# josebeo2016/SCL-Deepfake-audio-detection

Hardware: AMD Instinct MI355X
Metric: train-step utterances/sec (64000-sample clips) (higher is better)
Workload: dtype bf16

## Files before the change

scl-deepfake-audio-detection_amd/csrc/conv0.hip:

```cpp
#include "common.h"

namespace {

constexpr int MAXK = 16;
constexpr int MAXCH0 = 2;

struct Conv0Smem {
    float* wT;
    float* xs;
    float* red;
};

__device__ __forceinline__ void conv0_stage(float* wT, float* xs, const float* __restrict__ w, const float* __restrict__ x,
                                            int C, int k, int L, int x0, int nx) {
    for (int i = threadIdx.x; i < C * k; i += blockDim.x) {
        const int c = i / k, j = i % k;
        wT[j * C + c] = w[i];
    }
    for (int i = threadIdx.x; i < nx; i += blockDim.x) xs[i] = (x0 + i) < L ? x[x0 + i] : 0.f;
}

template <bool ZF32, int KC>
__global__ __launch_bounds__(256) void conv0_fwd_kernel(const float* __restrict__ x, const float* __restrict__ w,
                                                        const float* __restrict__ bias, const float* __restrict__ gamma,
                                                        const float* __restrict__ beta, void* __restrict__ zv, float* __restrict__ stats,
                                                        int L, int T0, int C, int k, int stride, int rows_per_block, float eps) {
    extern __shared__ __attribute__((aligned(16))) float sm0[];
    float* wT = sm0;
    float* xs = sm0 + k * C;
    const int b = blockIdx.y;
    const int t0 = blockIdx.x * rows_per_block;
    const int nrows = min(rows_per_block, T0 - t0);
    const int nx = nrows * stride + k;
    conv0_stage(wT, xs, w, x + (int64_t)b * L, C, k, L, t0 * stride, nx);
    __syncthreads();
    const int lane = threadIdx.x & 63, wv = threadIdx.x >> 6;
    float bia[MAXCH0][8], gam[MAXCH0][8], bet[MAXCH0][8];
#pragma unroll
    for (int ch = 0; ch < MAXCH0; ++ch) {
        const int c = ch * 512 + lane * 8;
#pragma unroll
        for (int i = 0; i < 8; ++i) {
            bia[ch][i] = c < C ? bias[c + i] : 0.f; gam[ch][i] = c < C ? gamma[c + i] : 0.f; bet[ch][i] = c < C ? beta[c + i] : 0.f;
        }
    }
    for (int r = wv; r < nrows; r += 4) {
        float y[MAXCH0][8];
        float s = 0.f;
#pragma unroll
        for (int ch = 0; ch < MAXCH0; ++ch) {
            const int c = ch * 512 + lane * 8;
            if (c < C) {
#pragma unroll
                for (int i = 0; i < 8; ++i) y[ch][i] = bia[ch][i];
#pragma unroll
                for (int j = 0; j < (KC ? KC : k); ++j) {
                    const float xv = xs[r * stride + j];
                    const float4 w0 = *reinterpret_cast<const float4*>(wT + j * C + c);
                    const float4 w1 = *reinterpret_cast<const float4*>(wT + j * C + c + 4);
                    y[ch][0] += w0.x * xv; y[ch][1] += w0.y * xv; y[ch][2] += w0.z * xv; y[ch][3] += w0.w * xv;
                    y[ch][4] += w1.x * xv; y[ch][5] += w1.y * xv; y[ch][6] += w1.z * xv; y[ch][7] += w1.w * xv;
                }
#pragma unroll
                for (int i = 0; i < 8; ++i) s += y[ch][i];
            }
        }
        const float mean = wave_sum(s) / (float)C;
        float q = 0.f;
#pragma unroll
        for (int ch = 0; ch < MAXCH0; ++ch) {
            const int c = ch * 512 + lane * 8;
            if (c < C) {
#pragma unroll
                for (int i = 0; i < 8; ++i) { const float d = y[ch][i] - mean; q += d * d; }
            }
        }
        const float rstd = rsqrtf(wave_sum(q) / (float)C + eps);
        if (stats && lane == 0) {
            stats[2 * ((int64_t)b * T0 + t0 + r)] = mean;
            stats[2 * ((int64_t)b * T0 + t0 + r) + 1] = rstd;
        }
#pragma unroll
        for (int ch = 0; ch < MAXCH0; ++ch) {
            const int c = ch * 512 + lane * 8;
            if (c < C) {
                float o[8];
#pragma unroll
                for (int i = 0; i < 8; ++i) o[i] = (y[ch][i] - mean) * rstd * gam[ch][i] + bet[ch][i];
#pragma unroll
                for (int i = 0; i < 8; i += 2) gelu2(o[i], o[i + 1]);
                const int64_t off = ((int64_t)b * T0 + t0 + r) * C + c;
                if (ZF32) {
                    float* z = reinterpret_cast<float*>(zv);
                    *reinterpret_cast<float4*>(z + off) = make_float4(o[0], o[1], o[2], o[3]);
                    *reinterpret_cast<float4*>(z + off + 4) = make_float4(o[4], o[5], o[6], o[7]);
                } else {
                    uint4 u;
                    u.x = pack_bf2(o[0], o[1]); u.y = pack_bf2(o[2], o[3]); u.z = pack_bf2(o[4], o[5]); u.w = pack_bf2(o[6], o[7]);
                    *reinterpret_cast<uint4*>(reinterpret_cast<bf16_t*>(zv) + off) = u;
                }
            }
        }
    }
}

template <bool STATS, int KT, bool FULLK>
__global__ __launch_bounds__(256, 2) void conv0_bwd_kernel(const float* __restrict__ x, const float* __restrict__ w,
                                                           const float* __restrict__ bias, const float* __restrict__ gamma,
                                                           const float* __restrict__ beta, const bf16_t* __restrict__ dz,
                                                           const float* __restrict__ stats, float* __restrict__ part, int L, int T0, int C,
                                                           int k, int stride, int rows_per_block, float eps) {
    extern __shared__ __attribute__((aligned(16))) float sm0[];
    float* wT = sm0;
    float* xs = sm0 + k * C;
    float* red = sm0;
    const int b = blockIdx.y;
    const int t0 = blockIdx.x * rows_per_block;
    const int nrows = min(rows_per_block, T0 - t0);
    const int nx = nrows * stride + k;
    conv0_stage(wT, xs, w, x + (int64_t)b * L, C, k, L, t0 * stride, nx);
    __syncthreads();
    const int lane = threadIdx.x & 63, wv = threadIdx.x >> 6;
    float aw[8][KT + 3];
#pragma unroll
    for (int i = 0; i < 8; ++i)
#pragma unroll
        for (int q = 0; q < KT + 3; ++q) aw[i][q] = 0.f;
    const int c = lane * 8;
    const bool act = c < C;
    float gam[8], bet[8], bia[8];
#pragma unroll
    for (int i = 0; i < 8; ++i) { gam[i] = act ? gamma[c + i] : 0.f; bet[i] = act ? beta[c + i] : 0.f; bia[i] = act ? bias[c + i] : 0.f; }
    uint4 u_next = make_uint4(0, 0, 0, 0);
    float mean_next = 0.f, rstd_next = 0.f;
    if (wv < nrows) {
        const int64_t row0 = (int64_t)b * T0 + t0 + wv;
        if (act) u_next = *reinterpret_cast<const uint4*>(dz + row0 * C + c);
        if (STATS) { mean_next = stats[2 * row0]; rstd_next = stats[2 * row0 + 1]; }
    }
    for (int r = wv; r < nrows; r += 4) {
        float y[8], g8[8], dzv[8], xr[KT];
        const int64_t row = (int64_t)b * T0 + t0 + r;
        const uint4 u = u_next;
        const float mean_cur = mean_next, rstd_cur = rstd_next;
        if (r + 4 < nrows) {
            if (act) u_next = *reinterpret_cast<const uint4*>(dz + (row + 4) * C + c);
            if (STATS) { mean_next = stats[2 * (row + 4)]; rstd_next = stats[2 * (row + 4) + 1]; }
        }
#pragma unroll
        for (int j = 0; j < KT; ++j) xr[j] = (FULLK || j < k) ? xs[r * stride + j] : 0.f;
        if (act) {
#pragma unroll
            for (int i = 0; i < 8; ++i) y[i] = bia[i];
#pragma unroll
            for (int j = 0; j < KT; ++j) {
                if (j < k) {
                    const float4 w0 = *reinterpret_cast<const float4*>(wT + j * C + c);
                    const float4 w1 = *reinterpret_cast<const float4*>(wT + j * C + c + 4);
                    y[0] += w0.x * xr[j]; y[1] += w0.y * xr[j]; y[2] += w0.z * xr[j]; y[3] += w0.w * xr[j];
                    y[4] += w1.x * xr[j]; y[5] += w1.y * xr[j]; y[6] += w1.z * xr[j]; y[7] += w1.w * xr[j];
                }

            }
            const uint32_t uw[4] = {u.x, u.y, u.z, u.w};
#pragma unroll
            for (int i = 0; i < 4; ++i) { dzv[2 * i] = __uint_as_float(uw[i] << 16); dzv[2 * i + 1] = __uint_as_float(uw[i] & 0xFFFF0000u); }
        } else {
#pragma unroll
            for (int i = 0; i < 8; ++i) { y[i] = 0.f; dzv[i] = 0.f; }
        }
        float mean, rstd;
        if (STATS) {
            mean = mean_cur; rstd = rstd_cur;
        } else {
            float s = 0.f;
#pragma unroll
            for (int i = 0; i < 8; ++i) s += y[i];
            mean = wave_sum(s) / (float)C;
            float q = 0.f;
            if (act) {
#pragma unroll
                for (int i = 0; i < 8; ++i) { const float dd = y[i] - mean; q += dd * dd; }
            }
            rstd = rsqrtf(wave_sum(q) / (float)C + eps);
        }
        float s1 = 0.f, s2 = 0.f;
        if (act) {
            float gg[8];
#pragma unroll
            for (int i = 0; i < 8; ++i) gg[i] = ((y[i] - mean) * rstd) * gam[i] + bet[i];
#pragma unroll
            for (int i = 0; i < 8; i += 2) gelu_grad2(gg[i], gg[i + 1]);
#pragma unroll
            for (int i = 0; i < 8; ++i) {
                const float h = (y[i] - mean) * rstd;
                const float gmi = gam[i];
                const float dyn = dzv[i] * gg[i];
                aw[i][KT + 1] += dyn * h;
                aw[i][KT + 2] += dyn;
                const float dh = dyn * gmi;
                y[i] = h;
                g8[i] = dh;
                s1 += dh; s2 += dh * h;
            }
        }
        s1 = wave_sum(s1) / (float)C;
        s2 = wave_sum(s2) / (float)C;
        if (act) {
#pragma unroll
            for (int i = 0; i < 8; ++i) {
                const float dy = rstd * (g8[i] - s1 - y[i] * s2);
                aw[i][KT] += dy;
#pragma unroll
                for (int j = 0; j < KT; ++j)
                    if (FULLK || j < k) aw[i][j] += dy * xr[j];
            }
        }
    }
    __syncthreads();
    for (int i = threadIdx.x; i < C * (k + 3); i += blockDim.x) red[i] = 0.f;
    __syncthreads();
    for (int ww = 0; ww < 4; ++ww) {
        if (wv == ww && act) {
#pragma unroll
            for (int i = 0; i < 8; ++i) {
#pragma unroll
                for (int j = 0; j < KT; ++j)
                    if (FULLK || j < k) red[(c + i) * (k + 3) + j] += aw[i][j];
                red[(c + i) * (k + 3) + k] += aw[i][KT];
                red[(c + i) * (k + 3) + k + 1] += aw[i][KT + 1];
                red[(c + i) * (k + 3) + k + 2] += aw[i][KT + 2];
            }
        }
        __syncthreads();
    }
    const int64_t blk = (int64_t)blockIdx.y * gridDim.x + blockIdx.x;
    for (int i = threadIdx.x; i < C * (k + 3); i += blockDim.x) part[blk * C * (k + 3) + i] = red[i];
}

__global__ void conv0_reduce_seg_kernel(float* __restrict__ part, int nparts, int n, int S) {
    const int i = blockIdx.x * blockDim.x + threadIdx.x;
    const int g = blockIdx.y;
    if (i >= n || g >= nparts) return;
    float s = 0.f;
    for (int p = g; p < nparts; p += S) s += part[(int64_t)p * n + i];
    part[(int64_t)g * n + i] = s;
}

__global__ void conv0_reduce_kernel(const float* __restrict__ part, int nparts, int C, int k, float* __restrict__ dW,
                                    float* __restrict__ db, float* __restrict__ dgamma, float* __restrict__ dbeta) {
    const int i = blockIdx.x * blockDim.x + threadIdx.x;
    const int n = C * (k + 3);
    if (i >= n) return;
    float s = 0.f;
    for (int p = 0; p < nparts; ++p) s += part[(int64_t)p * n + i];
    const int c = i / (k + 3), q = i % (k + 3);
    if (q < k) dW[c * k + q] = s;
    else if (q == k) db[c] = s;
    else if (q == k + 1) dgamma[c] = s;
    else dbeta[c] = s;
}

}

static int conv0_bwd_rows(int B, int T0) {
    int best_rows = 1024; long long best = -1;
    for (int chunks = (T0 + 1023) / 1024; chunks <= (T0 + 63) / 64; ++chunks) {
        const int rows = (T0 + chunks - 1) / chunks;
        const long long blocks = (long long)B * ((T0 + rows - 1) / rows);
        const long long cost = ((blocks + 511) / 512) * (rows + 48);
        if (best < 0 || cost < best) { best = cost; best_rows = rows; }
        if (blocks > 8192) break;
    }
    return best_rows < 64 ? 64 : best_rows;
}

extern "C" int scl_conv0_fwd(const float* x, const float* w, const float* bias, const float* gamma, const float* beta,
                             void* z, float* stats, int B, int L, int C, int k, int stride, float eps, void* stream) {
    SCL_REQUIRE(x && w && bias && gamma && beta && z, "conv0_fwd: null pointer");
    SCL_REQUIRE(B > 0 && L >= k && C >= 8 && C <= 1024 && (C & 7) == 0 && k >= 1 && k <= MAXK && stride >= 1, "conv0_fwd: bad dims");
    const int T0 = (L - k) / stride + 1;
    const int rows = 128;
    dim3 grid((T0 + rows - 1) / rows, B), block(256);
    const size_t lds = (size_t)(k * C + rows * stride + k) * sizeof(float);
    if (k == 10) hipLaunchKernelGGL((conv0_fwd_kernel<false, 10>), grid, block, lds, (hipStream_t)stream, x, w, bias, gamma, beta, z, stats, L, T0, C, k, stride, rows, eps);
    else hipLaunchKernelGGL((conv0_fwd_kernel<false, 0>), grid, block, lds, (hipStream_t)stream, x, w, bias, gamma, beta, z, stats, L, T0, C, k, stride, rows, eps);
    return scl_check_launch("scl_conv0_fwd");
}

extern "C" int scl_conv0_fwd_f32(const float* x, const float* w, const float* bias, const float* gamma, const float* beta,
                                 float* z, int B, int L, int C, int k, int stride, float eps, void* stream) {
    SCL_REQUIRE(x && w && bias && gamma && beta && z, "conv0_fwd_f32: null pointer");
    SCL_REQUIRE(B > 0 && L >= k && C >= 8 && C <= 1024 && (C & 7) == 0 && k >= 1 && k <= MAXK && stride >= 1, "conv0_fwd_f32: bad dims");
    const int T0 = (L - k) / stride + 1;
    const int rows = 128;
    dim3 grid((T0 + rows - 1) / rows, B), block(256);
    const size_t lds = (size_t)(k * C + rows * stride + k) * sizeof(float);
    if (k == 10) hipLaunchKernelGGL((conv0_fwd_kernel<true, 10>), grid, block, lds, (hipStream_t)stream, x, w, bias, gamma, beta, (void*)z, nullptr, L, T0, C, k, stride, rows, eps);
    else hipLaunchKernelGGL((conv0_fwd_kernel<true, 0>), grid, block, lds, (hipStream_t)stream, x, w, bias, gamma, beta, (void*)z, nullptr, L, T0, C, k, stride, rows, eps);
    return scl_check_launch("scl_conv0_fwd_f32");
}

extern "C" int scl_conv0_bwd_nparts(int B, int L, int k, int stride) {
    const int T0 = (L - k) / stride + 1;
    const int rows = conv0_bwd_rows(B, T0);
    return B * ((T0 + rows - 1) / rows);
}

extern "C" int scl_conv0_bwd(const float* x, const float* w, const float* bias, const float* gamma, const float* beta,
                             const void* dz, const float* stats, float* part_ws, float* dW, float* db, float* dgamma, float* dbeta,
                             int B, int L, int C, int k, int stride, float eps, void* stream) {
    SCL_REQUIRE(x && w && bias && gamma && beta && dz && part_ws && dW && db && dgamma && dbeta, "conv0_bwd: null pointer");
    SCL_REQUIRE(B > 0 && L >= k && C >= 8 && C <= 512 && (C & 7) == 0 && k >= 1 && k <= MAXK && stride >= 1, "conv0_bwd: bad dims (C <= 512)");
    const int T0 = (L - k) / stride + 1;
    const int rows = conv0_bwd_rows(B, T0);
    dim3 grid((T0 + rows - 1) / rows, B), block(256);
    const size_t a = (size_t)(k * C + rows * stride + k), r = (size_t)C * (k + 3);
    const size_t lds = (a > r ? a : r) * sizeof(float);
    hipStream_t s = (hipStream_t)stream;
#define CONV0_BWD(ST, KT, FK) hipLaunchKernelGGL((conv0_bwd_kernel<ST, KT, FK>), grid, block, lds, s, x, w, bias, gamma, beta, (const bf16_t*)dz, stats, \
                                                 part_ws, L, T0, C, k, stride, rows, eps)
    if (k == 10) { if (stats) CONV0_BWD(true, 10, true); else CONV0_BWD(false, 10, true); }
    else if (k < 10) { if (stats) CONV0_BWD(true, 10, false); else CONV0_BWD(false, 10, false); }
    else { if (stats) CONV0_BWD(true, MAXK, false); else CONV0_BWD(false, MAXK, false); }
#undef CONV0_BWD
    int nparts = grid.x * grid.y;
    const int n = C * (k + 3);
    if (nparts > 64) {
        const int S = 32;
        hipLaunchKernelGGL(conv0_reduce_seg_kernel, dim3((n + 255) / 256, S), dim3(256), 0, s, part_ws, nparts, n, S);
        nparts = S;
    }
    hipLaunchKernelGGL(conv0_reduce_kernel, dim3((n + 255) / 256), dim3(256), 0, s, part_ws, nparts, C, k, dW, db, dgamma, dbeta);
    return scl_check_launch("scl_conv0_bwd");
}
```

Measured before the change: 1633.

## Add MFMA-based conv0 forward and backward kernels with fused LayerNorm and GELU

Adds new first-layer conv kernels for forward and backward that compute the k-tap convolution as fp32 MFMA 16x16x4 matrix ops, using a rearranged weight layout in shared memory. LayerNorm, GELU and the parameter gradients stay fused in the same kernel. The backward kernel splits channels across waves and exchanges row sums through LDS, and the forward picks its row tiling from a cost model. This moves conv0 work off scalar FMAs onto the matrix units. The path is on by default and can be turned off with an environment variable. It adds a lot of code and uses an erf approximation for GELU, which carries some numerical risk.

```diff
diff --git a/scl-deepfake-audio-detection_amd/csrc/conv0.hip b/scl-deepfake-audio-detection_amd/csrc/conv0.hip
--- a/scl-deepfake-audio-detection_amd/csrc/conv0.hip
+++ b/scl-deepfake-audio-detection_amd/csrc/conv0.hip
@@ -1,3 +1,4 @@
+#include <stdlib.h>
 #include "common.h"
 
 namespace {
@@ -105,7 +106,7 @@
 }
 
 template <bool STATS, int KT, bool FULLK>
-__global__ __launch_bounds__(256, 2) void conv0_bwd_kernel(const float* __restrict__ x, const float* __restrict__ w,
+__global__ __launch_bounds__(256, KT > 10 ? 1 : 2) void conv0_bwd_kernel(const float* __restrict__ x, const float* __restrict__ w,
                                                            const float* __restrict__ bias, const float* __restrict__ gamma,
                                                            const float* __restrict__ beta, const bf16_t* __restrict__ dz,
                                                            const float* __restrict__ stats, float* __restrict__ part, int L, int T0, int C,
@@ -261,6 +262,361 @@
     else dbeta[c] = s;
 }
 
+constexpr int C0M_PAD = 16;
+
+__device__ __forceinline__ int conv0m_channel(int t, int n) { return 128 * (t >> 3) + 8 * n + (t & 7); }
+__device__ __forceinline__ int conv0m_slab(int rows, int stride) { return ((rows + 15) & ~15) * stride + C0M_PAD; }
+
+__device__ __forceinline__ void conv0m_stage(float* wB, float* xs, const float* __restrict__ w, const float* __restrict__ x,
+                                             int C, int k, int nm, int L, int x0, int nx) {
+    const int nt4 = C >> 6;
+    for (int i = threadIdx.x; i < nm * C * 4; i += blockDim.x) {
+        const int e = i & 3, ln = (i >> 2) & 63, rest = i >> 8;
+        const int t = 4 * (rest % nt4) + e, m = rest / nt4;
+        const int tap = 4 * m + (ln >> 4);
+        wB[i] = tap < k ? w[conv0m_channel(t, ln & 15) * k + tap] : 0.f;
+    }
+    for (int i = threadIdx.x; i < nx; i += blockDim.x) xs[i] = (x0 + i) < L ? x[x0 + i] : 0.f;
+}
+
+template <int NV>
+__device__ __forceinline__ void conv0m_gelu_parts(const float (&x)[NV], float (&cdf)[NV], float (&e)[NV]) {
+#pragma clang fp contract(off)
+    typedef __attribute__((ext_vector_type(NV))) float vec;
+    vec xv, ax, t, ev;
+#pragma unroll
+    for (int i = 0; i < NV; ++i) { xv[i] = x[i]; ax[i] = fabsf(x[i]); }
+    const vec z = ax * 0.70710678118654752f;
+    const vec den = __builtin_elementwise_fma(vec(0.3275911f), z, vec(1.0f));
+#pragma unroll
+    for (int i = 0; i < NV; ++i) t[i] = __builtin_amdgcn_rcpf(den[i]);
+    const vec z2 = z * z;
+#pragma unroll
+    for (int i = 0; i < NV; ++i) ev[i] = __expf(-z2[i]);
+    vec p = __builtin_elementwise_fma(t, vec(1.061405429f), vec(-1.453152027f));
+    p = __builtin_elementwise_fma(t, p, vec(1.421413741f));
+    p = __builtin_elementwise_fma(t, p, vec(-0.284496736f));
+    p = __builtin_elementwise_fma(t, p, vec(0.254829592f));
+    const vec half_tail = (0.5f * (t * p)) * ev;
+#pragma unroll
+    for (int i = 0; i < NV; ++i) { cdf[i] = x[i] >= 0.f ? 1.0f - half_tail[i] : half_tail[i]; e[i] = ev[i]; }
+}
+template <int NV>
+__device__ __forceinline__ void conv0m_gelu(float (&x)[NV]) {
+    float cdf[NV], e[NV];
+    conv0m_gelu_parts<NV>(x, cdf, e);
+#pragma unroll
+    for (int i = 0; i < NV; ++i) x[i] = x[i] * cdf[i];
+}
+template <int NV>
+__device__ __forceinline__ void conv0m_gelu_grad(float (&x)[NV]) {
+#pragma clang fp contract(off)
+    float cdf[NV], e[NV];
+    conv0m_gelu_parts<NV>(x, cdf, e);
+#pragma unroll
+    for (int i = 0; i < NV; ++i) x[i] = __builtin_fmaf(x[i] * 0.39894228040143268f, e[i], cdf[i]);
+}
+
+template <bool ZF32, int NC, int KM>
+__global__ __launch_bounds__(256, 2) void conv0_fwd_mfma_kernel(const float* __restrict__ x, const float* __restrict__ w,
+                                                                const float* __restrict__ bias, const float* __restrict__ gamma,
+                                                                const float* __restrict__ beta, void* __restrict__ zv,
+                                                                float* __restrict__ stats, int L, int T0, int k, int stride,
+                                                                int rows_per_block, float eps) {
+    constexpr int C = 128 * NC, NT = 8 * NC;
+    extern __shared__ __attribute__((aligned(16))) float sm0[];
+    constexpr int nm = KM;
+    float* wB = sm0;
+    float* aff = wB + nm * C * 4;
+    float* xs = aff + 3 * C;
+    const int b = blockIdx.y;
+    const int t0 = blockIdx.x * rows_per_block;
+    const int nrows = min(rows_per_block, T0 - t0);
+    conv0m_stage(wB, xs, w, x + (int64_t)b * L, C, k, nm, L, t0 * stride, conv0m_slab(rows_per_block, stride));
+    for (int i = threadIdx.x; i < C; i += blockDim.x) { aff[i] = bias[i]; aff[C + i] = gamma[i]; aff[2 * C + i] = beta[i]; }
+    __syncthreads();
+    const int lane = threadIdx.x & 63, wv = threadIdx.x >> 6;
+    const int n = lane & 15, g = lane >> 4;
+    const int ngroups = (nrows + 15) >> 4;
+    for (int grp = wv; grp < ngroups; grp += 4) {
+        f32x4 acc[NT];
+#pragma unroll
+        for (int q = 0; q < NC; ++q) {
+            const float4 b0 = *reinterpret_cast<const float4*>(aff + 128 * q + 8 * n);
+            const float4 b1 = *reinterpret_cast<const float4*>(aff + 128 * q + 8 * n + 4);
+            const float bb[8] = {b0.x, b0.y, b0.z, b0.w, b1.x, b1.y, b1.z, b1.w};
+#pragma unroll
+            for (int i = 0; i < 8; ++i) acc[8 * q + i] = f32x4{bb[i], bb[i], bb[i], bb[i]};
+        }
+        const float* xa = xs + stride * (16 * grp + n) + g;
+        const float4* wb = reinterpret_cast<const float4*>(wB) + lane;
+#pragma unroll 1
+        for (int m = 0; m < KM; ++m) {
+            const float a = xa[4 * m];
+#pragma unroll
+            for (int t4 = 0; t4 < NT / 4; ++t4) {
+                const float4 bv = wb[(m * (NT / 4) + t4) * 64];
+                acc[4 * t4 + 0] = __builtin_amdgcn_mfma_f32_16x16x4f32(a, bv.x, acc[4 * t4 + 0], 0, 0, 0);
+                acc[4 * t4 + 1] = __builtin_amdgcn_mfma_f32_16x16x4f32(a, bv.y, acc[4 * t4 + 1], 0, 0, 0);
+                acc[4 * t4 + 2] = __builtin_amdgcn_mfma_f32_16x16x4f32(a, bv.z, acc[4 * t4 + 2], 0, 0, 0);
+                acc[4 * t4 + 3] = __builtin_amdgcn_mfma_f32_16x16x4f32(a, bv.w, acc[4 * t4 + 3], 0, 0, 0);
+            }
+        }
+        float mean[4], rstd[4];
+#pragma unroll
+        for (int r = 0; r < 4; ++r) {
+            float s = 0.f;
+#pragma unroll
+            for (int t = 0; t < NT; ++t) s += acc[t][r];
+            mean[r] = lanes16_sum(s) / (float)C;
+        }
+#pragma unroll
+        for (int r = 0; r < 4; ++r) {
+            float q = 0.f;
+#pragma unroll
+            for (int t = 0; t < NT; ++t) { const float d = acc[t][r] - mean[r]; q += d * d; }
+            rstd[r] = rsqrtf(lanes16_sum(q) / (float)C + eps);
+        }
+        const int fl0 = 16 * grp + 4 * g;
+        const int64_t row0 = (int64_t)b * T0 + t0 + fl0;
+        if (stats && n == 0) {
+#pragma unroll
+            for (int r = 0; r < 4; ++r)
+                if (fl0 + r < nrows) *reinterpret_cast<float2*>(stats + 2 * (row0 + r)) = make_float2(mean[r], rstd[r]);
+        }
+#pragma unroll
+        for (int q = 0; q < NC; ++q) {
+            __builtin_amdgcn_sched_barrier(0);
+            const float4 g0 = *reinterpret_cast<const float4*>(aff + C + 128 * q + 8 * n);
+            const float4 g1 = *reinterpret_cast<const float4*>(aff + C + 128 * q + 8 * n + 4);
+            const float4 e0 = *reinterpret_cast<const float4*>(aff + 2 * C + 128 * q + 8 * n);
+            const float4 e1 = *reinterpret_cast<const float4*>(aff + 2 * C + 128 * q + 8 * n + 4);
+            const float gam[8] = {g0.x, g0.y, g0.z, g0.w, g1.x, g1.y, g1.z, g1.w};
+            const float bet[8] = {e0.x, e0.y, e0.z, e0.w, e1.x, e1.y, e1.z, e1.w};
+#pragma unroll
+            for (int r = 0; r < 4; ++r) {
+                float o[8];
+#pragma unroll
+                for (int i = 0; i < 8; ++i) o[i] = (acc[8 * q + i][r] - mean[r]) * rstd[r] * gam[i] + bet[i];
+                conv0m_gelu<8>(o);
+                if (fl0 + r < nrows) {
+                    const int64_t off = (row0 + r) * C + 128 * q + 8 * n;
+                    if (ZF32) {
+                        float* z = reinterpret_cast<float*>(zv);
+                        *reinterpret_cast<float4*>(z + off) = make_float4(o[0], o[1], o[2], o[3]);
+                        *reinterpret_cast<float4*>(z + off + 4) = make_float4(o[4], o[5], o[6], o[7]);
+                    } else {
+                        uint4 u;
+                        u.x = pack_bf2(o[0], o[1]); u.y = pack_bf2(o[2], o[3]); u.z = pack_bf2(o[4], o[5]); u.w = pack_bf2(o[6], o[7]);
+                        *reinterpret_cast<uint4*>(reinterpret_cast<bf16_t*>(zv) + off) = u;
+                    }
+                }
+            }
+        }
+    }
+}
+
+template <int NC, int KM>
+__global__ __launch_bounds__(64 * NC, 2) void conv0_bwd_mfma_kernel(const float* __restrict__ x, const float* __restrict__ w,
+                                                                    const float* __restrict__ bias, const float* __restrict__ gamma,
+                                                                    const float* __restrict__ beta, const bf16_t* __restrict__ dz,
+                                                                    const float* __restrict__ stats, float* __restrict__ part, int L,
+                                                                    int T0, int k, int stride, int rows_per_block) {
+    constexpr int C = 128 * NC;
+    extern __shared__ __attribute__((aligned(16))) float sm0[];
+    constexpr int nm = KM;
+    float* wB = sm0;
+    float* aff = wB + nm * C * 4;
+    float* ex = aff + 3 * C;
+    float* xs = ex + 2 * NC * 32;
+    const int b = blockIdx.y;
+    const int t0 = blockIdx.x * rows_per_block;
+    const int nrows = min(rows_per_block, T0 - t0);
+    conv0m_stage(wB, xs, w, x + (int64_t)b * L, C, k, nm, L, t0 * stride, conv0m_slab(rows_per_block, stride));
+    for (int i = threadIdx.x; i < C; i += blockDim.x) { aff[i] = bias[i]; aff[C + i] = gamma[i]; aff[2 * C + i] = beta[i]; }
+    __syncthreads();
+    const int lane = threadIdx.x & 63, wv = threadIdx.x >> 6;
+    const int n = lane & 15, g = lane >> 4;
+    const int cb = 128 * wv + 8 * n;
+    f32x4 dwT[8];
+    float adb[8], adg[8], adbe[8];
+#pragma unroll
+    for (int i = 0; i < 8; ++i) { dwT[i] = f32x4{0.f, 0.f, 0.f, 0.f}; adb[i] = 0.f; adg[i] = 0.f; adbe[i] = 0.f; }
+    const int ngroups = (nrows + 15) >> 4;
+    const int64_t rowb = (int64_t)b * T0 + t0;
+    uint4 u[4];
+    float2 st[4];
+#pragma unroll
+    for (int r = 0; r < 4; ++r) {
+        const int fl = 4 * g + r;
+        u[r] = make_uint4(0, 0, 0, 0); st[r] = make_float2(0.f, 0.f);
+        if (fl < nrows) {
+            u[r] = *reinterpret_cast<const uint4*>(dz + (rowb + fl) * C + cb);
+            st[r] = *reinterpret_cast<const float2*>(stats + 2 * (rowb + fl));
+        }
+    }
+    const float4* wb = reinterpret_cast<const float4*>(wB) + lane;
+    for (int grp = 0; grp < ngroups; ++grp) {
+        f32x4 y[8], d[8];
+        {
+            const float4 b0 = *reinterpret_cast<const float4*>(aff + cb), b1 = *reinterpret_cast<const float4*>(aff + cb + 4);
+            const float bia[8] = {b0.x, b0.y, b0.z, b0.w, b1.x, b1.y, b1.z, b1.w};
+#pragma unroll
+            for (int i = 0; i < 8; ++i) y[i] = f32x4{bia[i], bia[i], bia[i], bia[i]};
+        }
+        const float* xa = xs + stride * (16 * grp + n) + g;
+#pragma unroll 1
+        for (int m = 0; m < KM; ++m) {
+            const float a = xa[4 * m];
+            const float4 b0 = wb[(m * 2 * NC + 2 * wv) * 64], b1 = wb[(m * 2 * NC + 2 * wv + 1) * 64];
+            y[0] = __builtin_amdgcn_mfma_f32_16x16x4f32(a, b0.x, y[0], 0, 0, 0);
+            y[1] = __builtin_amdgcn_mfma_f32_16x16x4f32(a, b0.y, y[1], 0, 0, 0);
+            y[2] = __builtin_amdgcn_mfma_f32_16x16x4f32(a, b0.z, y[2], 0, 0, 0);
+            y[3] = __builtin_amdgcn_mfma_f32_16x16x4f32(a, b0.w, y[3], 0, 0, 0);
+            y[4] = __builtin_amdgcn_mfma_f32_16x16x4f32(a, b1.x, y[4], 0, 0, 0);
+            y[5] = __builtin_amdgcn_mfma_f32_16x16x4f32(a, b1.y, y[5], 0, 0, 0);
+            y[6] = __builtin_amdgcn_mfma_f32_16x16x4f32(a, b1.z, y[6], 0, 0, 0);
+            y[7] = __builtin_amdgcn_mfma_f32_16x16x4f32(a, b1.w, y[7], 0, 0, 0);
+        }
+        float s1[4], s2[4];
+#pragma unroll
+        for (int r = 0; r < 4; ++r) {
+            __builtin_amdgcn_sched_barrier(0);
+            const float mean = st[r].x, rstd = st[r].y;
+            const float4 g0 = *reinterpret_cast<const float4*>(aff + C + cb), g1 = *reinterpret_cast<const float4*>(aff + C + cb + 4);
+            const float4 e0 = *reinterpret_cast<const float4*>(aff + 2 * C + cb), e1 = *reinterpret_cast<const float4*>(aff + 2 * C + cb + 4);
+            const float gam[8] = {g0.x, g0.y, g0.z, g0.w, g1.x, g1.y, g1.z, g1.w};
+            const float bet[8] = {e0.x, e0.y, e0.z, e0.w, e1.x, e1.y, e1.z, e1.w};
+            const uint32_t uw[4] = {u[r].x, u[r].y, u[r].z, u[r].w};
+            float dzv[8], gg[8];
+#pragma unroll
+            for (int i = 0; i < 4; ++i) { dzv[2 * i] = __uint_as_float(uw[i] << 16); dzv[2 * i + 1] = __uint_as_float(uw[i] & 0xFFFF0000u); }
+#pragma unroll
+            for (int i = 0; i < 8; ++i) gg[i] = ((y[i][r] - mean) * rstd) * gam[i] + bet[i];
+            conv0m_gelu_grad<8>(gg);
+            float a1 = 0.f, a2 = 0.f;
+#pragma unroll
+            for (int i = 0; i < 8; ++i) {
+                const float h = (y[i][r] - mean) * rstd;
+                const float dyn = dzv[i] * gg[i];
+                adg[i] += dyn * h;
+                adbe[i] += dyn;
+                const float dh = dyn * gam[i];
+                y[i][r] = h;
+                d[i][r] = dh;
+                a1 += dh; a2 += dh * h;
+            }
+            s1[r] = lanes16_sum(a1);
+            s2[r] = lanes16_sum(a2);
+        }
+        if (NC > 1) {
+            float* exb = ex + (grp & 1) * NC * 32;
+            if (n == 0) {
+#pragma unroll
+                for (int r = 0; r < 4; ++r) *reinterpret_cast<float2*>(exb + (wv * 16 + 4 * g + r) * 2) = make_float2(s1[r], s2[r]);
+            }
+            __syncthreads();
+#pragma unroll
+            for (int r = 0; r < 4; ++r) {
+                float t1 = 0.f, t2 = 0.f;
+#pragma unroll
+                for (int ww = 0; ww < NC; ++ww) {
+                    const float2 p = *reinterpret_cast<const float2*>(exb + (ww * 16 + 4 * g + r) * 2);
+                    t1 += p.x; t2 += p.y;
+                }
+                s1[r] = t1; s2[r] = t2;
+            }
+        }
+#pragma unroll
+        for (int r = 0; r < 4; ++r) {
+            const float rstd = st[r].y;
+            const float m1 = s1[r] / (float)C, m2 = s2[r] / (float)C;
+#pragma unroll
+            for (int i = 0; i < 8; ++i) {
+                const float dy = rstd * (d[i][r] - m1 - y[i][r] * m2);
+                adb[i] += dy;
+                d[i][r] = dy;
+            }
+        }
+#pragma unroll
+        for (int r = 0; r < 4; ++r) {
+            const int fl = 16 * (grp + 1) + 4 * g + r;
+            u[r] = make_uint4(0, 0, 0, 0); st[r] = make_float2(0.f, 0.f);
+            if (fl < nrows) {
+                u[r] = *reinterpret_cast<const uint4*>(dz + (rowb + fl) * C + cb);
+                st[r] = *reinterpret_cast<const float2*>(stats + 2 * (rowb + fl));
+            }
+        }
+        const float* xt = xs + stride * (16 * grp + 4 * g) + n;
+        __builtin_amdgcn_sched_barrier(0);
+#pragma unroll
+        for (int i = 0; i < 8; ++i) y[i] = f32x4{0.f, 0.f, 0.f, 0.f};
+#pragma unroll
+        for (int r = 0; r < 4; ++r) {
+            const float a = xt[stride * r];
+#pragma unroll
+            for (int i = 0; i < 8; ++i) y[i] = __builtin_amdgcn_mfma_f32_16x16x4f32(a, d[i][r], y[i], 0, 0, 0);
+        }
+#pragma unroll
+        for (int i = 0; i < 8; ++i) dwT[i] += y[i];
+    }
+#pragma unroll
+    for (int i = 0; i < 8; ++i) {
+        adb[i] += __shfl_xor(adb[i], 16); adb[i] += __shfl_xor(adb[i], 32);
+        adg[i] += __shfl_xor(adg[i], 16); adg[i] += __shfl_xor(adg[i], 32);
+        adbe[i] += __shfl_xor(adbe[i], 16); adbe[i] += __shfl_xor(adbe[i], 32);
+    }
+    float* prow = part + ((int64_t)blockIdx.y * gridDim.x + blockIdx.x) * C * (k + 3);
+#pragma unroll
+    for (int i = 0; i < 8; ++i) {
+        float* pc = prow + (cb + i) * (k + 3);
+#pragma unroll
+        for (int e = 0; e < 4; ++e)
+            if (4 * g + e < k) pc[4 * g + e] = dwT[i][e];
+        if (g == 0) { pc[k] = adb[i]; pc[k + 1] = adg[i]; pc[k + 2] = adbe[i]; }
+    }
+}
+
+}
+
+static bool conv0_use_mfma(int C, int k, size_t lds) {
+    static const bool on = [] { const char* e = getenv("SCL_CONV0_MFMA"); return !(e && atoi(e) == 0); }();
+    return on && C % 128 == 0 && C <= 512 && k <= MAXK && lds <= 64 * 1024;
+}
+static size_t conv0m_lds(int C, int k, int rows, int stride, int extra_floats) {
+    const int nm = (k + 3) / 4;
+    return ((size_t)nm * C * 4 + 3 * C + extra_floats + (size_t)((rows + 15) & ~15) * stride + C0M_PAD) * sizeof(float);
+}
+
+template <bool ZF32>
+static void conv0_fwd_mfma_launch(dim3 grid, size_t lds, hipStream_t s, const float* x, const float* w, const float* bias, const float* gamma,
+                                  const float* beta, void* z, float* stats, int L, int T0, int C, int k, int stride, int rows, float eps) {
+#define CONV0M_FWD(NC, KM) \
+    hipLaunchKernelGGL((conv0_fwd_mfma_kernel<ZF32, NC, KM>), grid, dim3(256), lds, s, x, w, bias, gamma, beta, z, stats, L, T0, k, stride, rows, eps)
+#define CONV0M_FWD_K(NC)                                          \
+    switch ((k + 3) / 4) {                                        \
+        case 1: CONV0M_FWD(NC, 1); break;                         \
+        case 2: CONV0M_FWD(NC, 2); break;                         \
+        case 3: CONV0M_FWD(NC, 3); break;                         \
+        default: CONV0M_FWD(NC, 4); break;                        \
+    }
+    switch (C / 128) {
+        case 1: CONV0M_FWD_K(1); break;
+        case 2: CONV0M_FWD_K(2); break;
+        case 3: CONV0M_FWD_K(3); break;
+        default: CONV0M_FWD_K(4); break;
+    }
+#undef CONV0M_FWD_K
+#undef CONV0M_FWD
+}
+static int conv0m_fwd_rows(int B, int T0) {
+    int best_rows = 64; long long best = -1;
+    for (int rows = 64; rows <= 512; rows += 64) {
+        const long long blocks = (long long)B * ((T0 + rows - 1) / rows);
+        const long long cost = ((blocks + 511) / 512) * (rows + 32);
+        if (best < 0 || cost < best) { best = cost; best_rows = rows; }
+    }
+    return best_rows;
 }
 
 static int conv0_bwd_rows(int B, int T0) {
@@ -280,6 +636,12 @@
     SCL_REQUIRE(x && w && bias && gamma && beta && z, "conv0_fwd: null pointer");
     SCL_REQUIRE(B > 0 && L >= k && C >= 8 && C <= 1024 && (C & 7) == 0 && k >= 1 && k <= MAXK && stride >= 1, "conv0_fwd: bad dims");
     const int T0 = (L - k) / stride + 1;
+    const int mrows = conv0m_fwd_rows(B, T0);
+    if (const size_t mlds = conv0m_lds(C, k, mrows, stride, 0); conv0_use_mfma(C, k, mlds)) {
+        conv0_fwd_mfma_launch<false>(dim3((T0 + mrows - 1) / mrows, B), mlds, (hipStream_t)stream, x, w, bias, gamma, beta, z, stats,
+                                     L, T0, C, k, stride, mrows, eps);
+        return scl_check_launch("scl_conv0_fwd");
+    }
     const int rows = 128;
     dim3 grid((T0 + rows - 1) / rows, B), block(256);
     const size_t lds = (size_t)(k * C + rows * stride + k) * sizeof(float);
@@ -293,6 +655,12 @@
     SCL_REQUIRE(x && w && bias && gamma && beta && z, "conv0_fwd_f32: null pointer");
     SCL_REQUIRE(B > 0 && L >= k && C >= 8 && C <= 1024 && (C & 7) == 0 && k >= 1 && k <= MAXK && stride >= 1, "conv0_fwd_f32: bad dims");
     const int T0 = (L - k) / stride + 1;
+    const int mrows = conv0m_fwd_rows(B, T0);
+    if (const size_t mlds = conv0m_lds(C, k, mrows, stride, 0); conv0_use_mfma(C, k, mlds)) {
+        conv0_fwd_mfma_launch<true>(dim3((T0 + mrows - 1) / mrows, B), mlds, (hipStream_t)stream, x, w, bias, gamma, beta, (void*)z, nullptr,
+                                    L, T0, C, k, stride, mrows, eps);
+        return scl_check_launch("scl_conv0_fwd_f32");
+    }
     const int rows = 128;
     dim3 grid((T0 + rows - 1) / rows, B), block(256);
     const size_t lds = (size_t)(k * C + rows * stride + k) * sizeof(float);
@@ -320,10 +688,29 @@
     hipStream_t s = (hipStream_t)stream;
 #define CONV0_BWD(ST, KT, FK) hipLaunchKernelGGL((conv0_bwd_kernel<ST, KT, FK>), grid, block, lds, s, x, w, bias, gamma, beta, (const bf16_t*)dz, stats, \
                                                  part_ws, L, T0, C, k, stride, rows, eps)
+#define CONV0M_BWD_K(NC, KM) \
+    hipLaunchKernelGGL((conv0_bwd_mfma_kernel<NC, KM>), grid, dim3(64 * NC), mlds, s, x, w, bias, gamma, beta, (const bf16_t*)dz, stats, part_ws, L, T0, k, stride, rows)
+#define CONV0M_BWD(NC)                                            \
+    switch ((k + 3) / 4) {                                        \
+        case 1: CONV0M_BWD_K(NC, 1); break;                       \
+        case 2: CONV0M_BWD_K(NC, 2); break;                       \
+        case 3: CONV0M_BWD_K(NC, 3); break;                       \
+        default: CONV0M_BWD_K(NC, 4); break;                      \
+    }
+    if (const size_t mlds = conv0m_lds(C, k, rows, stride, 2 * (C / 128) * 32); stats && conv0_use_mfma(C, k, mlds)) {
+        switch (C / 128) {
+            case 1: CONV0M_BWD(1); break;
+            case 2: CONV0M_BWD(2); break;
+            case 3: CONV0M_BWD(3); break;
+            default: CONV0M_BWD(4); break;
+        }
+    } else
     if (k == 10) { if (stats) CONV0_BWD(true, 10, true); else CONV0_BWD(false, 10, true); }
     else if (k < 10) { if (stats) CONV0_BWD(true, 10, false); else CONV0_BWD(false, 10, false); }
     else { if (stats) CONV0_BWD(true, MAXK, false); else CONV0_BWD(false, MAXK, false); }
 #undef CONV0_BWD
+#undef CONV0M_BWD
+#undef CONV0M_BWD_K
     int nparts = grid.x * grid.y;
     const int n = C * (k + 3);
     if (nparts > 64) {
```

After: 1648 (median of 6 runs). About the same (+0.9%).
